# hwwang55/GraphGAN

Hardware: NVIDIA H100
Metric: sampled negative edges/sec (D-sampling pass) (higher is better)
Workload: dtype f32

## Files before the change

### graphgan_b200/csrc/walk.cu

```cuda
#include <string.h>

#include "walk_common.cuh"

namespace gg {
namespace {

struct Rng {
    int mode;
    uint32_t k0, k1, tag;
    const double *stream;
    long long n_stream;
    long long cursor;
    int exhausted;
    __device__ __forceinline__ double draw(uint32_t root, uint32_t walk, uint32_t step) {
        if (mode == GG_RNG_PHILOX) {
            uint32_t a, b;
            philox4x32_10(root, walk, step, tag, k0, k1, a, b);
            return u53(a, b);
        }
        if (cursor >= n_stream) { exhausted = 1; return 0.0; }
        return stream[cursor++];
    }
};

// ... 260 lines not shown
#define GG_S1_SINGLES 65536
#endif
constexpr int S1_SINGLES = GG_S1_SINGLES, S1_CHUNK = 16;

template <int CPL>
__global__ void __launch_bounds__(WARPS_PER_CTA * 32, WALK_MIN_CTAS) step1_cdf_kernel(const __grid_constant__ gg_walk_desc d) {
    extern __shared__ __align__(16) unsigned char walk_smem[];
    const int lane = threadIdx.x & 31, wid = threadIdx.x >> 5;
    float *s_sc = reinterpret_cast<float *>(walk_smem + (size_t)wid * WALK_SMEM_PER_WARP);
    int *s_ids = reinterpret_cast<int *>(s_sc + SC_CAP);
    Stage stg;
    stg.buf = s_sc;
    stg.bar = reinterpret_cast<unsigned long long *>(s_ids + ID_CAP);
    stg.phase = 0u;
    stg.on = !d.no_tma && d.edge_score != nullptr;
    if (stg.on) {
        if (lane == 0) {
            mbar_init(stg.bar, 1);
            asm volatile("fence.mbarrier_init.release.cluster;" ::: "memory");
        }
        __syncwarp();
    }
    const long long gw = (long long)blockIdx.x * WARPS_PER_CTA + wid;
    const long long nwarps = (long long)gridDim.x * WARPS_PER_CTA;
    int *g_ids = reinterpret_cast<int *>(d.scratch) + (size_t)gw * 2 * (size_t)d.max_cand;
    float *g_sc = reinterpret_cast<float *>(g_ids + d.max_cand);
    unsigned long long rows_gathered = 0;
    unsigned int cyc[7] = {0, 0, 0, 0, 0, 0, 0};
    long long item = gw, sub = 0, sub_end = 0;
    const long long n_single = d.s1_nq < S1_SINGLES ? d.s1_nq : S1_SINGLES;
    const long long n_items = n_single + (d.s1_nq - n_single + S1_CHUNK - 1) / S1_CHUNK;
    for (;;) {
        long long pos;
        if (d.s1_order) {
            if (sub >= sub_end) {
                unsigned int it = 0;
                if (lane == 0) it = atomicAdd(d.work_counter, 1u);
                it = __shfl_sync(FULL, it, 0);
                if ((long long)it >= n_items) break;
                if ((long long)it < n_single) { sub = it; sub_end = sub + 1; }
                else { sub = n_single + ((long long)it - n_single) * S1_CHUNK; sub_end = sub + S1_CHUNK < d.s1_nq ? sub + S1_CHUNK : d.s1_nq; }
            }
            pos = __ldg(d.s1_order + sub);
            ++sub;
        } else {
            if (item >= d.s1_nq) break;
            pos = item;
            item += nwarps;
        }
        if (!s1_is_shared(d, pos)) continue;
        const int slot = __ldg(d.s1_slot + pos);
        const int root = d.roots[slot];
        const uint32_t *tb = d.tree_bits + (size_t)slot * (size_t)d.tree_words;
        const long long e = d.indptr[root] + (pos - __ldg(d.rq_ptr + slot));
        const int c = __ldg(d.adj + e);
        const bool inc_father = !d.for_d && !((d.d1_bits[e >> 5] >> (e & 31)) & 1u);
        int n; float m; int *ids; float *sc;
        build_list<CPL, UNR_S1>(d, tb, c, root, inc_father, s_ids, s_sc, g_ids, g_sc, lane, n, m, ids, sc, rows_gathered, cyc, stg);
        if (lane == 0) d.s1_n[pos] = n;
        if (n == 0) continue;
        const long long o = __ldg(d.s1_ptr + pos);
        for (int i = lane; i < n; i += 32) d.s1_ids[o + i] = ids[i];
        if (n > 1) cdf_store_raw<UNR_S1>(sc, n, m, d.s1_q + o, lane);
        __syncwarp();
    }
    if (lane == 0 && rows_gathered) atomicAdd(d.counters + GG_CNT_ROWS_GATHERED, rows_gathered);
}

struct FlatView {
    int4 *list[2];
    int4 *tail;
    int *hub;
    int *item_n;
    int *pool_ids;
    unsigned *ctr;
    int stride;
    int steps;
    unsigned long long *keys;
    int *owner;
    int *rec_slot;
    int *uniq;
    double *pool_cdf;
    unsigned long long tbl_mask;
};
constexpr int FLAT_MAX_STEPS = 14;
constexpr int FLAT_CTR_WORDS = 1 + 4 * (FLAT_MAX_STEPS + 2);
#define GG_FCTR(fv, s, k) ((fv).ctr + 1 + 4 * (s) + (k))
__device__ __forceinline__ int4 *level_list(const FlatView &fv, int s) { return (s & 1) ? fv.list[1] : fv.list[0]; }

#ifndef GG_SHARE_LEVELS
#define GG_SHARE_LEVELS 0x4
#endif
constexpr unsigned SHARE_LEVELS = (unsigned)(GG_SHARE_LEVELS) & ~3u;
__host__ __device__ constexpr bool level_shared(int s) { return s < 32 && ((SHARE_LEVELS >> s) & 1u); }
inline bool any_level_shared(int steps) { return steps >= 2 && (SHARE_LEVELS & ((steps >= 31 ? ~0u : ((2u << steps) - 1u)))) != 0; }

template <int CPL>
__global__ void __launch_bounds__(WARPS_PER_CTA * 32, WALK_MIN_CTAS) walk_kernel(const __grid_constant__ gg_walk_desc d,
                                                                                 const FlatView fv, const int tail_mode) {
    extern __shared__ __align__(16) unsigned char walk_smem[];
    const int lane = threadIdx.x & 31, wid = threadIdx.x >> 5;
    float *s_sc = reinterpret_cast<float *>(walk_smem + (size_t)wid * WALK_SMEM_PER_WARP);
    int *s_ids = reinterpret_cast<int *>(s_sc + SC_CAP);
    Stage stg;
    stg.buf = s_sc;
    stg.bar = reinterpret_cast<unsigned long long *>(s_ids + ID_CAP);
    stg.phase = 0u;
    stg.on = !d.no_tma && d.edge_score != nullptr;
    if (stg.on) {
        if (lane == 0) {
            mbar_init(stg.bar, 1);
            asm volatile("fence.mbarrier_init.release.cluster;" ::: "memory");
        }
        __syncwarp();
    }
    const long long gw = (long long)blockIdx.x * WARPS_PER_CTA + wid;
    int *g_ids = reinterpret_cast<int *>(d.scratch) + (size_t)gw * 2 * (size_t)d.max_cand;
    float *g_sc = reinterpret_cast<float *>(g_ids + d.max_cand);
    Rng rng;
    rng.mode = GG_RNG_PHILOX; rng.k0 = (uint32_t)d.seed; rng.k1 = (uint32_t)(d.seed >> 32); rng.tag = d.pass_tag;
    rng.stream = nullptr; rng.n_stream = 0; rng.cursor = 0; rng.exhausted = 0;
    unsigned long long raw_steps = 0, raw_suml = 0, overflow = 0, rows_gathered = 0;
    unsigned int cyc[7] = {0, 0, 0, 0, 0, 0, 0};
    const bool ratio_all = d.update_ratio >= 1.0;

    const long long n_items = tail_mode ? (long long)fv.ctr[0] : d.n_walks;
    for (;;) {
        unsigned int wi = 0;
        if (lane == 0) wi = atomicAdd(d.work_counter, 1u);
        wi = __shfl_sync(FULL, wi, 0);
        if ((long long)wi >= n_items) break;
        if (tail_mode) {
            const int4 rec = fv.tail[wi];
            const long long w = rec.x;
            const int slot = rec.w;
            WalkState from;
            from.cur = rec.y; from.prev = rec.z; from.step = d.wsteps[w]; from.fedge = d.first_edge[w]; from.suml = d.wsuml[w];
            walk_one<CPL>(d, rng, slot, (uint32_t)(w - __ldg(d.walk_ptr + slot)), w, s_ids, s_sc, g_ids, g_sc, lane, raw_steps,
                          raw_suml, overflow, rows_gathered, cyc, stg, &from);
            continue;
        }
        const long long w = d.walk_order ? (long long)__ldg(d.walk_order + wi) : (long long)wi;
        int slot;
        if (d.walk_slot) {
            slot = __ldg(d.walk_slot + w);
        } else {
            long long lo = 0, hi = d.n_roots;
            while (hi - lo > 1) {
                const long long mid = (lo + hi) >> 1;
                if (__ldg(d.walk_ptr + mid) <= w) lo = mid; else hi = mid;
            }
            slot = (int)lo;
        }
        const uint32_t k = (uint32_t)(w - __ldg(d.walk_ptr + slot));
        if (!ratio_all) {
            uint32_t a, b;
            philox4x32_10((uint32_t)d.roots[slot], 0xffffffffu, 0u, rng.tag, rng.k0, rng.k1, a, b);
            if (!(u53(a, b) < d.update_ratio)) {
                if (lane == 0) {
                    d.samples[w] = -1; d.status[w] = GG_SKIPPED; d.first_edge[w] = -1; d.wsteps[w] = 0; d.wsuml[w] = 0;
                    if (d.path_len) d.path_len[w] = 0;
                }
                continue;
            }
        }
        walk_one<CPL>(d, rng, slot, k, w, s_ids, s_sc, g_ids, g_sc, lane, raw_steps, raw_suml, overflow, rows_gathered,
                      cyc, stg);
    }
    if (lane == 0) {
#pragma unroll
        for (int q = 0; q < 7; ++q) if (cyc[q]) atomicAdd(d.counters + GG_CNT_CYC_ENUM + q, (unsigned long long)cyc[q]);
        if (raw_steps) atomicAdd(d.counters + GG_CNT_RAW_STEPS, raw_steps);
        if (raw_suml) atomicAdd(d.counters + GG_CNT_RAW_SUML, raw_suml);
        if (overflow) atomicAdd(d.counters + GG_CNT_PATH_OVERFLOW, overflow);
        if (rows_gathered) atomicAdd(d.counters + GG_CNT_ROWS_GATHERED, rows_gathered);
    }
}

// ... 54 lines not shown
                status = GG_VOID;
            } else {
                const long long a0 = d.indptr[root];
                const int n0 = (int)(d.indptr[root + 1] - a0);
                fedge = (int)(a0 + fi);
                const int c = __ldg(d.adj + fedge);
                if (prow && 1 < d.max_path) prow[1] = c;
                ws = 1; wl = n0; steps = 1; suml = (unsigned)n0;
                const long long s1pos = __ldg(d.rq_ptr + slot) + fi;
                if (s1_is_shared(d, s1pos)) {
                    const int n = __ldg(d.s1_n + s1pos);
                    if (n == 0) {
                        status = GG_VOID;
                    } else {
                        const bool inc_father = step_includes_father(d, 1, fedge);
                        const long long o = __ldg(d.s1_ptr + s1pos);
                        uint32_t a, b;
                        philox4x32_10((uint32_t)root, k, 1u, d.pass_tag, (uint32_t)d.seed, (uint32_t)(d.seed >> 32), a, b);
                        const int idx = (n == 1) ? 0 : cdf_search_raw(d.s1_q + o, n, u53(a, b));
                        const int nxt = __ldg(d.s1_ids + o + idx);
                        if (prow && 2 < d.max_path) prow[2] = nxt;
                        ws = 2; wl = n0 + n; steps = 2; suml = (unsigned)(n0 + n);
                        if (inc_father && idx == 0) {
                            sample = c; status = GG_DONE; plen = 3;
                            if (d.max_path > 0 && 3 > d.max_path) over = 1;
                        } else {
                            rec = make_int4((int)w, nxt, c, slot); dest = 2;
                        }
                    }
                } else {
                    rec = make_int4((int)w, c, root, slot); dest = 1;
                }
            }
        }
        d.samples[w] = sample; d.status[w] = status; d.first_edge[w] = fedge; d.wsteps[w] = ws; d.wsuml[w] = wl;
        if (d.path_len) d.path_len[w] = plen;
    }
#pragma unroll
    for (int lv = 1; lv <= 2; ++lv) {
        const unsigned mk = __ballot_sync(FULL, dest == lv);
        if (!mk) continue;
        const int leader = __ffs(mk) - 1;
        int4 *list = (lv <= fv.steps) ? fv.list[lv & 1] : fv.tail;
        unsigned *cnt = (lv <= fv.steps) ? GG_FCTR(fv, lv, 0) : fv.ctr;
        unsigned base = 0;
        if (lane == leader) base = atomicAdd(cnt, (unsigned)__popc(mk));
        base = __shfl_sync(FULL, base, leader);
        if (dest == lv) list[base + __popc(mk & ((1u << lane) - 1u))] = rec;
    }
    steps = __reduce_add_sync(FULL, steps); suml = __reduce_add_sync(FULL, suml); over = __reduce_add_sync(FULL, over);
    if (lane == 0) {
        if (steps) atomicAdd(d.counters + GG_CNT_RAW_STEPS, (unsigned long long)steps);
        if (suml) atomicAdd(d.counters + GG_CNT_RAW_SUML, (unsigned long long)suml);
        if (over) atomicAdd(d.counters + GG_CNT_PATH_OVERFLOW, (unsigned long long)over);
    }
}

__device__ __forceinline__ unsigned long long share_hash(unsigned long long key, unsigned long long mask) {
    return ((key * 0x9E3779B97F4A7C15ull) >> 20) & mask;
}

template <class T>
__device__ __forceinline__ void warp_append(bool take, T *list, unsigned *cnt, const T &v, int lane) {
    const unsigned mk = __ballot_sync(FULL, take);
    if (!mk) return;
    const int leader = __ffs(mk) - 1;
    unsigned base = 0;
    if (lane == leader) base = atomicAdd(cnt, (unsigned)__popc(mk));
    base = __shfl_sync(FULL, base, leader);
    if (take) list[base + __popc(mk & ((1u << lane) - 1u))] = v;
}

__global__ void __launch_bounds__(256) flat_dedupe_kernel(const __grid_constant__ gg_walk_desc d, const FlatView fv, const int s) {
    const unsigned i = blockIdx.x * blockDim.x + threadIdx.x;
    const int lane = threadIdx.x & 31;
    const unsigned nA = *GG_FCTR(fv, s, 0);
    if (blockIdx.x * blockDim.x >= nA) return;
    bool hub = false, owner = false;
    if (i < nA) {
        const int4 rec = level_list(fv, s)[i];
        const int cur = rec.y, slot = rec.w;
        hub = d.edge_score && (d.indptr[cur + 1] - d.indptr[cur]) >= d.hub_threshold;
        int h = -1;
        if (!hub) {
            const unsigned long long key = (unsigned long long)slot * (unsigned long long)d.n_node + (unsigned long long)cur;
            unsigned long long p = share_hash(key, fv.tbl_mask);
            for (;;) {
                const unsigned long long old = atomicCAS(fv.keys + p, ~0ull, key);
                if (old == ~0ull) { owner = true; fv.owner[p] = (int)i; break; }
                if (old == key) break;
                p = (p + 1) & fv.tbl_mask;
            }
            h = (int)p;
        }
        fv.rec_slot[i] = h;
    }
    const int item = (int)i;
    warp_append(hub, fv.hub, GG_FCTR(fv, s, 1), item, lane);
    warp_append(owner, fv.uniq, GG_FCTR(fv, s, 2), item, lane);
}

__global__ void __launch_bounds__(256) flat_draw_kernel(const __grid_constant__ gg_walk_desc d, const FlatView fv, const int s) {
    const unsigned i = blockIdx.x * blockDim.x + threadIdx.x;
    const int lane = threadIdx.x & 31;
    const unsigned nA = *GG_FCTR(fv, s, 0);
    if (blockIdx.x * blockDim.x >= nA) return;
    unsigned long long overflow = 0;
    unsigned steps = 0, suml = 0;
    bool go_on = false;
    int4 rec = make_int4(0, 0, 0, 0);
    if (i < nA) {
        const int h = fv.rec_slot[i];
        if (h >= 0) {
            rec = level_list(fv, s)[i];
            const long long w = rec.x;
            const int cur = rec.y, slot = rec.w;
            const int item = fv.owner[h];
            const int nrec = fv.item_n[item];
            const int n = nrec & 0x3fffffff;
            if (n == 0) {
                flat_void(d, s, w);
            } else {
                const bool inc_father = (nrec >> 30) & 1;
                int idx = 0;
                if (n > 1) {
                    uint32_t a, b;
                    philox4x32_10((uint32_t)d.roots[slot], (uint32_t)(w - __ldg(d.walk_ptr + slot)), (uint32_t)s, d.pass_tag,
                                  (uint32_t)d.seed, (uint32_t)(d.seed >> 32), a, b);
                    idx = cdf_search_raw(fv.pool_cdf + (size_t)item * (size_t)(fv.stride + 1), n, u53(a, b));
                }
                const int nxt = fv.pool_ids[(size_t)item * (size_t)fv.stride + idx];
                go_on = flat_record_choice(d, s, w, cur, n, idx, nxt, inc_father, overflow);
                rec = make_int4((int)w, nxt, cur, slot);
                steps = 1; suml = (unsigned)n;
            }
        }
    }
    if (s < fv.steps) warp_append(go_on, level_list(fv, s + 1), GG_FCTR(fv, s + 1, 0), rec, lane);
    else warp_append(go_on, fv.tail, fv.ctr, rec, lane);
    steps = __reduce_add_sync(FULL, steps); suml = __reduce_add_sync(FULL, suml);
    const unsigned over = __reduce_add_sync(FULL, (unsigned)overflow);
    if (lane == 0) {
        if (steps) atomicAdd(d.counters + GG_CNT_RAW_STEPS, (unsigned long long)steps);
        if (suml) atomicAdd(d.counters + GG_CNT_RAW_SUML, (unsigned long long)suml);
        if (over) atomicAdd(d.counters + GG_CNT_PATH_OVERFLOW, (unsigned long long)over);
    }
}

constexpr int FLAT_ENUM_WARPS = 8;
template <bool SHARED>
__global__ void __launch_bounds__(FLAT_ENUM_WARPS * 32, 6) flat_enum_kernel(const __grid_constant__ gg_walk_desc d,
                                                                            const FlatView fv, const int s) {
    const int lane = threadIdx.x & 31;
    const unsigned gw = blockIdx.x * FLAT_ENUM_WARPS + (threadIdx.x >> 5), nwarps = gridDim.x * FLAT_ENUM_WARPS;
    const int4 *A = level_list(fv, s);
    const unsigned nA = SHARED ? *GG_FCTR(fv, s, 2) : *GG_FCTR(fv, s, 0);
    Stage stg;
    stg.buf = nullptr; stg.bar = nullptr; stg.phase = 0u; stg.on = false;
    unsigned long long raw_steps = 0, raw_suml = 0, overflow = 0;
    int4 rec_next = (gw < nA) ? A[SHARED ? fv.uniq[gw] : gw] : make_int4(0, 0, 0, 0);
    for (unsigned j = gw; j < nA; j += nwarps) {
        const unsigned i = SHARED ? (unsigned)fv.uniq[j] : j;
        const int4 rec = rec_next;
        if (j + nwarps < nA) rec_next = A[SHARED ? fv.uniq[j + nwarps] : j + nwarps];
        const long long w = rec.x;
        const int cur = rec.y, prev = rec.z, slot = rec.w;
        const long long a0 = d.indptr[cur], a1 = d.indptr[cur + 1];
        if (!SHARED && d.edge_score && (a1 - a0) >= d.hub_threshold) {
            if (lane == 0) { fv.hub[atomicAdd(GG_FCTR(fv, s, 1), 1u)] = (int)i; fv.item_n[i] = 0; }
            continue;
        }
        const bool inc_father = step_includes_father(d, s, s == 1 ? d.first_edge[w] : 0);
        const uint32_t *tb = d.tree_bits + (size_t)slot * (size_t)d.tree_words;
        int *ids = fv.pool_ids + (size_t)i * (size_t)fv.stride;
        int n = 0;
        if (inc_father) { if (lane == 0) ids[0] = prev; n = 1; }
        float m = 0.0f;
        enumerate_children<UNR>(d, tb, a0, a1, false, ids, nullptr, lane, n, m, stg);
        __syncwarp();
        if (SHARED) {
            if (lane == 0) fv.item_n[i] = n | (inc_father ? (1 << 30) : 0);
        } else if (n == 0) {
            if (lane == 0) { flat_void(d, s, w); fv.item_n[i] = 0; }
        } else if (n == 1) {
            const int nxt = inc_father ? prev : ids[0];
            if (lane == 0) { flat_advance(d, fv, s, w, slot, cur, 1, 0, nxt, inc_father, overflow); fv.item_n[i] = 0; }
            raw_steps += 1; raw_suml += 1;
        } else if (lane == 0) {
            fv.item_n[i] = n | (inc_father ? (1 << 30) : 0);
        }
    }
    if (lane == 0) {
        if (raw_steps) atomicAdd(d.counters + GG_CNT_RAW_STEPS, raw_steps);
        if (raw_suml) atomicAdd(d.counters + GG_CNT_RAW_SUML, raw_suml);
        if (overflow) atomicAdd(d.counters + GG_CNT_PATH_OVERFLOW, overflow);
    }
}

template <int CPL, bool SHARED>
__global__ void __launch_bounds__(WARPS_PER_CTA * 32, WALK_MIN_CTAS) flat_choose_kernel(const __grid_constant__ gg_walk_desc d,
                                                                                        const FlatView fv, const int s) {
    extern __shared__ __align__(16) unsigned char walk_smem[];
    const int lane = threadIdx.x & 31, wid = threadIdx.x >> 5;
    float *s_sc = reinterpret_cast<float *>(walk_smem + (size_t)wid * WALK_SMEM_PER_WARP);
    int *s_ids = reinterpret_cast<int *>(s_sc + SC_CAP);
    Stage stg;
    stg.buf = s_sc;
    stg.bar = reinterpret_cast<unsigned long long *>(s_ids + ID_CAP);
    stg.phase = 0u;
    stg.on = !d.no_tma && d.edge_score != nullptr;
    if (stg.on) {
        if (lane == 0) {
            mbar_init(stg.bar, 1);
            asm volatile("fence.mbarrier_init.release.cluster;" ::: "memory");
        }
        __syncwarp();
    }
    const long long gw = (long long)blockIdx.x * WARPS_PER_CTA + wid;
    int *g_ids = reinterpret_cast<int *>(d.scratch) + (size_t)gw * 2 * (size_t)d.max_cand;
    float *g_sc = reinterpret_cast<float *>(g_ids + d.max_cand);
    const int4 *A = level_list(fv, s);
    const unsigned nA = SHARED ? *GG_FCTR(fv, s, 2) : *GG_FCTR(fv, s, 0), nH = *GG_FCTR(fv, s, 1);
    const uint32_t k0 = (uint32_t)d.seed, k1 = (uint32_t)(d.seed >> 32);
    unsigned long long raw_steps = 0, raw_suml = 0, overflow = 0, rows_gathered = 0;
    unsigned int cyc[7] = {0, 0, 0, 0, 0, 0, 0};
    constexpr unsigned FLAT_CHUNK = 8;
    const unsigned n_pulls = nH + (nA + FLAT_CHUNK - 1) / FLAT_CHUNK;
    for (;;) {
        unsigned j = 0;
        if (lane == 0) j = atomicAdd(GG_FCTR(fv, s, 3), 1u);
        j = __shfl_sync(FULL, j, 0);
        if (j >= n_pulls) break;
        const bool hub_item = j < nH;
        unsigned p = hub_item ? 0u : (j - nH) * FLAT_CHUNK;
        const unsigned p_end = hub_item ? 1u : ((p + FLAT_CHUNK < nA) ? p + FLAT_CHUNK : nA);
        unsigned i_next = hub_item ? (unsigned)fv.hub[j] : (SHARED ? (unsigned)fv.uniq[p] : p);
        int4 rec_next = A[i_next];
        int n_next = hub_item ? 0 : fv.item_n[i_next];
        for (; p < p_end; ++p) {
            const unsigned i = i_next;
            const int4 rec = rec_next;
            const int nrec = n_next;
            if (p + 1 < p_end) {
                i_next = SHARED ? (unsigned)fv.uniq[p + 1] : p + 1;
                rec_next = A[i_next]; n_next = fv.item_n[i_next];
            }
            if (!hub_item && (nrec & 0x3fffffff) < 2) continue;
            const long long w = rec.x;
            const int cur = rec.y, prev = rec.z, slot = rec.w;
            int n, idx, nxt;
            bool inc_father;
            uint32_t a, b;
            if (hub_item) {
                inc_father = step_includes_father(d, s, s == 1 ? d.first_edge[w] : 0);
                const uint32_t *tb = d.tree_bits + (size_t)slot * (size_t)d.tree_words;
                int *ids; float *sc; float m;
                build_list<CPL, UNR>(d, tb, cur, prev, inc_father, s_ids, s_sc, g_ids, g_sc, lane, n, m, ids, sc, rows_gathered, cyc, stg);
                if (n == 0) {
                    if (lane == 0) flat_void(d, s, w);
                    continue;
                }
                philox4x32_10((uint32_t)d.roots[slot], (uint32_t)(w - __ldg(d.walk_ptr + slot)), (uint32_t)s, d.pass_tag, k0, k1, a, b);
                idx = (n == 1) ? 0 : choose_index(sc, n, m, u53(a, b), lane, sc != s_sc ? reinterpret_cast<double *>(s_sc) : nullptr);
                nxt = ids[idx];
                __syncwarp();
            } else {
                n = nrec & 0x3fffffff;
                inc_father = (nrec >> 30) & 1;
                const int *ids = fv.pool_ids + (size_t)i * (size_t)fv.stride;
                float4 c4[CPL];
                load_row<CPL>(d.emb, d.ld, cur, lane & 7, c4);
                const int root = d.roots[slot];
                const uint32_t k = (uint32_t)(w - __ldg(d.walk_ptr + slot));
                score_list<CPL>(d.emb, d.bias, d.ld, c4, ids, s_sc, n, cur, lane);
                rows_gathered += 1u + (unsigned)n;
                const float m = list_max(s_sc, n, lane);
                if (SHARED) {
                    cdf_store_raw<UNR>(s_sc, n, m, fv.pool_cdf + (size_t)i * (size_t)(fv.stride + 1), lane);
                    __syncwarp();
                    continue;
                }
                philox4x32_10((uint32_t)root, k, (uint32_t)s, d.pass_tag, k0, k1, a, b);
                idx = choose_index(s_sc, n, m, u53(a, b), lane);
                nxt = ids[idx];
                __syncwarp();
            }
            if (lane == 0) {
                flat_advance(d, fv, s, w, slot, cur, n, idx, nxt, inc_father, overflow);
                raw_steps += 1; raw_suml += (unsigned)n;
            }
        }
    }
    if (lane == 0) {
        if (raw_steps) atomicAdd(d.counters + GG_CNT_RAW_STEPS, raw_steps);
        if (raw_suml) atomicAdd(d.counters + GG_CNT_RAW_SUML, raw_suml);
        if (overflow) atomicAdd(d.counters + GG_CNT_PATH_OVERFLOW, overflow);
        if (rows_gathered) atomicAdd(d.counters + GG_CNT_ROWS_GATHERED, rows_gathered);
    }
}

size_t flat_layout(void *buf, long long n_walks, int hub_threshold, int steps, FlatView *fv) {
    const size_t W = (size_t)(n_walks > 0 ? n_walks : 1);
    const int stride = ((hub_threshold > 0 ? hub_threshold : 1) + 31) / 32 * 32;
    size_t off = 0;
    auto take = [&](size_t bytes) {
        void *p = buf ? (void *)((unsigned char *)buf + off) : nullptr;
        off += (bytes + 255) & ~(size_t)255;
        return p;
    };
    unsigned *ctr = (unsigned *)take(sizeof(unsigned) * FLAT_CTR_WORDS);
    int4 *l0 = (int4 *)take(16 * W), *l1 = (int4 *)take(16 * W), *tail = (int4 *)take(16 * W);
    int *hub = (int *)take(4 * W), *item_n = (int *)take(4 * W);
    int *pool = (int *)take(4 * W * (size_t)stride);
    unsigned long long cap = 0;
    unsigned long long *keys = nullptr;
    int *owner = nullptr, *rec_slot = nullptr, *uniq = nullptr;
    double *cdf = nullptr;
    if (any_level_shared(steps)) {
        cap = 1;
        while (cap < 2 * (unsigned long long)W) cap <<= 1;
        keys = (unsigned long long *)take(8 * cap);
        owner = (int *)take(4 * cap);
        rec_slot = (int *)take(4 * W);
        uniq = (int *)take(4 * W);
        cdf = (double *)take(8 * W * (size_t)(stride + 1));
    }
    if (fv) {
        fv->ctr = ctr; fv->list[0] = l0; fv->list[1] = l1; fv->tail = tail; fv->hub = hub;
        fv->item_n = item_n; fv->pool_ids = pool; fv->stride = stride; fv->steps = steps;
        fv->keys = keys; fv->owner = owner; fv->rec_slot = rec_slot; fv->uniq = uniq; fv->pool_cdf = cdf;
        fv->tbl_mask = cap ? cap - 1 : 0;
    }
    return off;
}

template <int CPL>
__global__ void __launch_bounds__(32) walk_stream_kernel(const __grid_constant__ gg_walk_desc d) {
    extern __shared__ __align__(16) unsigned char walk_smem[];
    float *s_sc = reinterpret_cast<float *>(walk_smem);
    int *s_ids = reinterpret_cast<int *>(s_sc + SC_CAP);
    const int lane = threadIdx.x;
    int *g_ids = reinterpret_cast<int *>(d.scratch);
    float *g_sc = reinterpret_cast<float *>(g_ids + d.max_cand);
    Rng rng;
    rng.mode = GG_RNG_STREAM; rng.k0 = rng.k1 = rng.tag = 0;
    rng.stream = d.stream; rng.n_stream = d.n_stream; rng.cursor = 0; rng.exhausted = 0;
    unsigned long long raw_steps = 0, raw_suml = 0, overflow = 0, rows_gathered = 0;
    unsigned int cyc[7] = {0, 0, 0, 0, 0, 0, 0};
    Stage stg;
    stg.buf = s_sc; stg.bar = nullptr; stg.phase = 0u; stg.on = false;
    for (long long slot = 0; slot < d.n_roots && !rng.exhausted; ++slot) {
        const long long w0 = d.walk_ptr[slot], w1 = d.walk_ptr[slot + 1];
        const double ur = rng.draw(0, 0, 0);
        const bool skip = !(ur < d.update_ratio);
        bool dead = skip || rng.exhausted;
        for (long long w = w0; w < w1; ++w) {
            if (dead) {
                if (lane == 0) {
                    d.samples[w] = -1; d.status[w] = skip ? GG_SKIPPED : GG_NOTRUN; d.first_edge[w] = -1;
                    d.wsteps[w] = 0; d.wsuml[w] = 0;
                    if (d.path_len) d.path_len[w] = 0;
                }
                continue;
            }
            const int st = walk_one<CPL>(d, rng, (int)slot, (uint32_t)(w - w0), w, s_ids, s_sc, g_ids, g_sc, lane,
                                         raw_steps, raw_suml, overflow, rows_gathered, cyc, stg);
            if (st != GG_DONE) dead = true;
        }
    }
    if (lane == 0) {
        atomicAdd(d.counters + GG_CNT_RAW_STEPS, raw_steps);
        atomicAdd(d.counters + GG_CNT_RAW_SUML, raw_suml);
        atomicAdd(d.counters + GG_CNT_PATH_OVERFLOW, overflow);
        atomicAdd(d.counters + GG_CNT_ROWS_GATHERED, rows_gathered);
        d.counters[GG_CNT_STREAM_USED] = (unsigned long long)rng.cursor + (rng.exhausted ? (1ull << 62) : 0ull);
    }
}

constexpr int FIN_NONE = 0x7f7f7f7f;

__device__ __forceinline__ long long walk_root_slot(const long long *__restrict__ walk_ptr, long long n_roots, long long w) {
    long long lo = 0, hi = n_roots;
    while (hi - lo > 1) {
        const long long mid = (lo + hi) >> 1;
        if (__ldg(walk_ptr + mid) <= w) lo = mid; else hi = mid;
    }
    return lo;
}

__global__ void finalize_mark_kernel(long long n_roots, const long long *__restrict__ walk_ptr, const int *__restrict__ status,
                                     int *root_ok) {
    const long long W = walk_ptr[n_roots];
    for (long long w = (long long)blockIdx.x * blockDim.x + threadIdx.x; w < W; w += (long long)gridDim.x * blockDim.x) {
        if (status[w] == GG_DONE) continue;
        const long long slot = walk_root_slot(walk_ptr, n_roots, w);
        atomicMin(root_ok + slot, (int)(w - walk_ptr[slot]));
    }
}

__global__ void finalize_apply_kernel(long long n_roots, const long long *__restrict__ walk_ptr, int for_d, int *samples,
                                      int *status, const int *__restrict__ first_edge, int *wsteps, int *wsuml, int *path_len,
                                      uint32_t *d1_bits, const int *__restrict__ root_ok, unsigned long long *counters) {
    const long long W = walk_ptr[n_roots];
    unsigned long long steps = 0, suml = 0;
    for (long long w = (long long)blockIdx.x * blockDim.x + threadIdx.x; w < W; w += (long long)gridDim.x * blockDim.x) {
        const long long slot = walk_root_slot(walk_ptr, n_roots, w);
        const long long off = w - walk_ptr[slot];
        if (off <= (long long)root_ok[slot]) {
            steps += (unsigned)wsteps[w]; suml += (unsigned)wsuml[w];
            if (for_d && status[w] == GG_DONE) {
                const int fe = first_edge[w];
                if (fe >= 0) atomicOr(d1_bits + (fe >> 5), 1u << (fe & 31));
            }
        } else {
// ... 71 lines not shown
    *bytes = (int64_t)gg::flat_layout(nullptr, n_walks, hub_threshold, flat_steps, nullptr);
    return 0;
}

extern "C" int gg_walk_sample(const gg_walk_desc *dp, void *stream) {
    GG_REQUIRE(dp, "null descriptor");
    const gg_walk_desc &d = *dp;
    GG_REQUIRE(d.ld > 0 && d.ld % 32 == 0, "ld must be a positive multiple of 32");
    if (d.n_walks == 0 || d.n_roots == 0) return 0;
    GG_REQUIRE(d.emb && d.bias && d.indptr && d.adj && d.roots && d.tree_bits && d.walk_ptr, "null graph/embedding pointer");
    GG_REQUIRE(d.tree_words > 0, "tree_words missing (gg_tree_words)");
    GG_REQUIRE(d.samples && d.status && d.first_edge && d.wsteps && d.wsuml && d.counters && d.work_counter,
               "null output pointer");
    GG_REQUIRE(d.for_d || d.d1_bits, "G mode needs d1_bits");
    GG_REQUIRE(d.n_walks < (1ll << 32), "too many walks in one call");
    GG_REQUIRE(d.max_cand > 0 && d.scratch, "scratch missing");
    GG_REQUIRE(!d.root_q || d.rq_ptr, "root_q needs rq_ptr");
    GG_REQUIRE(d.max_path >= 0 && (d.max_path == 0 || (d.paths && d.path_len)), "max_path > 0 needs paths and path_len");
    GG_REQUIRE(d.phase_mask >= 0 && d.phase_mask <= 3, "phase_mask must be 0..3");
    GG_REQUIRE(d.update_ratio >= 0.0, "update_ratio must be >= 0");
    GG_REQUIRE(d.rng_mode == GG_RNG_PHILOX || d.rng_mode == GG_RNG_STREAM, "unknown rng_mode");
    {
        const bool any_s1 = d.s1_q || d.s1_ids || d.s1_cnt || d.s1_n || d.s1_ptr || d.s1_slot || d.first_idx || d.s1_order;
        GG_REQUIRE(!any_s1 || (d.s1_q && d.s1_ids && d.s1_cnt && d.s1_n && d.s1_ptr && d.s1_slot && d.first_idx && d.s1_nq > 0),
                   "depth-1 reuse: s1_q, s1_ids, s1_cnt, s1_n, s1_ptr, s1_slot, first_idx and s1_nq go together");
        GG_REQUIRE(!any_s1 || d.rng_mode == GG_RNG_PHILOX, "depth-1 reuse needs GG_RNG_PHILOX");
        GG_REQUIRE(!d.walk_order || d.rng_mode == GG_RNG_PHILOX, "walk_order needs GG_RNG_PHILOX");
    }
    GG_REQUIRE(!d.edge_score || (d.hub_threshold > 0 && d.hub_threshold < gg::SMEM_CAP), "hub_threshold out of range");
    cudaStream_t st = (cudaStream_t)stream;
    GG_CHECK(cudaMemsetAsync(d.work_counter, 0, sizeof(unsigned int), st));
    if (d.n_walks == 0 || d.n_roots == 0) return 0;
    const int cpl = d.ld / 32;
    if (d.rng_mode == GG_RNG_STREAM) {
        GG_REQUIRE(d.stream, "stream mode needs the uniform stream");
        GG_REQUIRE(d.scratch_bytes >= 2ll * d.max_cand * 4, "scratch too small");
        switch (cpl) {
#define GG_STREAM(C)                                                                                                  \
    GG_CHECK(cudaFuncSetAttribute(gg::walk_stream_kernel<C>, cudaFuncAttributeMaxDynamicSharedMemorySize,            \
                                  gg::WALK_SMEM_PER_WARP));                                                          \
    gg::walk_stream_kernel<C><<<1, 32, gg::WALK_SMEM_PER_WARP, st>>>(d)
            case 1: GG_STREAM(1); break;
            case 2: GG_STREAM(2); break;
            case 4: GG_STREAM(4); break;
            case 8: GG_STREAM(8); break;
#undef GG_STREAM
            default: gg::set_error("gg_walk_sample: unsupported ld %d (supported: 32, 64, 128, 256)", d.ld); return 2;
        }
    } else {
        const int ctas = gg::grid_ctas();
        GG_REQUIRE(d.scratch_bytes >= (int64_t)ctas * gg::WARPS_PER_CTA * 2 * d.max_cand * 4, "scratch too small");
        const int pm = d.phase_mask ? d.phase_mask : 3;
        if (d.s1_q && (pm & 1)) {
            GG_REQUIRE(d.root_q && d.walk_slot && d.first_idx && d.s1_cnt && d.s1_n && d.s1_ptr && d.s1_ids && d.s1_slot,
                       "depth-1 reuse needs root_q, walk_slot and the s1_* buffers");
            GG_CHECK(cudaMemsetAsync(d.s1_cnt, 0, sizeof(int32_t) * (size_t)d.s1_nq, st));
            gg::root_step_kernel<<<(unsigned)((d.n_walks + 255) / 256), 256, 0, st>>>(d);
            GG_CHECK(cudaGetLastError());
#define GG_S1(C)                                                                                                      \
    GG_CHECK(cudaFuncSetAttribute(gg::step1_cdf_kernel<C>, cudaFuncAttributeMaxDynamicSharedMemorySize,              \
                                  gg::WARPS_PER_CTA * gg::WALK_SMEM_PER_WARP));                                      \
    gg::step1_cdf_kernel<C><<<ctas, gg::WARPS_PER_CTA * 32, gg::WARPS_PER_CTA * gg::WALK_SMEM_PER_WARP, st>>>(d)
            switch (cpl) {
                case 1: GG_S1(1); break;
                case 2: GG_S1(2); break;
                case 4: GG_S1(4); break;
                case 8: GG_S1(8); break;
                default: gg::set_error("gg_walk_sample: unsupported ld %d (supported: 32, 64, 128, 256)", d.ld); return 2;
            }
#undef GG_S1
            GG_CHECK(cudaGetLastError());
            GG_CHECK(cudaMemsetAsync(d.work_counter, 0, sizeof(unsigned int), st));
        }
        if (!(pm & 2)) return 0;
        gg::FlatView fv;
        memset(&fv, 0, sizeof(fv));
        int tail_mode = 0;
        if (d.flat_steps > 0) {
            GG_REQUIRE(d.s1_q && d.edge_score && d.root_q && d.walk_slot && d.first_idx, "flat_steps needs the depth-1 reuse (s1_*, edge_score, root_q, walk_slot)");
            GG_REQUIRE(d.flat_steps <= gg::FLAT_MAX_STEPS, "flat_steps too large");
            GG_REQUIRE(d.flat_buf && d.flat_bytes >= (int64_t)gg::flat_layout(nullptr, d.n_walks, d.hub_threshold, d.flat_steps, nullptr),
                       "flat_buf too small (gg_walk_flat_bytes)");
            gg::flat_layout(d.flat_buf, d.n_walks, d.hub_threshold, d.flat_steps, &fv);
            GG_CHECK(cudaMemsetAsync(fv.ctr, 0, sizeof(unsigned) * gg::FLAT_CTR_WORDS, st));
            gg::flat_start_kernel<<<(unsigned)((d.n_walks + 255) / 256), 256, 0, st>>>(d, fv);
            GG_CHECK(cudaGetLastError());
            const int enum_ctas = gg::sm_count() * 8;
            const unsigned rec_ctas = (unsigned)((d.n_walks + 255) / 256);
            GG_REQUIRE(!gg::any_level_shared(d.flat_steps) || d.n_node > 0, "n_node missing");
            for (int s = 1; s <= d.flat_steps; ++s) {
                const bool shared = gg::level_shared(s);
                if (shared) {
                    GG_CHECK(cudaMemsetAsync(fv.keys, 0xff, sizeof(unsigned long long) * (size_t)(fv.tbl_mask + 1), st));
                    gg::flat_dedupe_kernel<<<rec_ctas, 256, 0, st>>>(d, fv, s);
                    GG_CHECK(cudaGetLastError());
                    gg::flat_enum_kernel<true><<<enum_ctas, gg::FLAT_ENUM_WARPS * 32, 0, st>>>(d, fv, s);
                } else {
                    gg::flat_enum_kernel<false><<<enum_ctas, gg::FLAT_ENUM_WARPS * 32, 0, st>>>(d, fv, s);
                }
                GG_CHECK(cudaGetLastError());
                switch (cpl) {
#define GG_FLAT(C)                                                                                                    \
    if (shared) {                                                                                                    \
        GG_CHECK(cudaFuncSetAttribute(gg::flat_choose_kernel<C, true>, cudaFuncAttributeMaxDynamicSharedMemorySize,  \
                                      gg::WARPS_PER_CTA * gg::WALK_SMEM_PER_WARP));                                  \
        gg::flat_choose_kernel<C, true><<<ctas, gg::WARPS_PER_CTA * 32, gg::WARPS_PER_CTA * gg::WALK_SMEM_PER_WARP, st>>>(d, fv, s); \
    } else {                                                                                                         \
        GG_CHECK(cudaFuncSetAttribute(gg::flat_choose_kernel<C, false>, cudaFuncAttributeMaxDynamicSharedMemorySize, \
                                      gg::WARPS_PER_CTA * gg::WALK_SMEM_PER_WARP));                                  \
        gg::flat_choose_kernel<C, false><<<ctas, gg::WARPS_PER_CTA * 32, gg::WARPS_PER_CTA * gg::WALK_SMEM_PER_WARP, st>>>(d, fv, s); \
    }
                    case 1: GG_FLAT(1); break;
                    case 2: GG_FLAT(2); break;
                    case 4: GG_FLAT(4); break;
                    case 8: GG_FLAT(8); break;
#undef GG_FLAT
                    default: gg::set_error("gg_walk_sample: unsupported ld %d (supported: 32, 64, 128, 256)", d.ld); return 2;
                }
                GG_CHECK(cudaGetLastError());
                if (shared) {
                    gg::flat_draw_kernel<<<rec_ctas, 256, 0, st>>>(d, fv, s);
                    GG_CHECK(cudaGetLastError());
                }
            }
            tail_mode = 1;
        }
        switch (cpl) {
#define GG_WALK(C)                                                                                                    \
    GG_CHECK(cudaFuncSetAttribute(gg::walk_kernel<C>, cudaFuncAttributeMaxDynamicSharedMemorySize,                   \
                                  gg::WARPS_PER_CTA * gg::WALK_SMEM_PER_WARP));                                      \
    gg::walk_kernel<C><<<ctas, gg::WARPS_PER_CTA * 32, gg::WARPS_PER_CTA * gg::WALK_SMEM_PER_WARP, st>>>(d, fv, tail_mode)
            case 1: GG_WALK(1); break;
            case 2: GG_WALK(2); break;
            case 4: GG_WALK(4); break;
            case 8: GG_WALK(8); break;
#undef GG_WALK
            default: gg::set_error("gg_walk_sample: unsupported ld %d (supported: 32, 64, 128, 256)", d.ld); return 2;
        }
    }
    return gg::check_cuda(cudaGetLastError(), "walk kernel launch");
}

extern "C" int gg_walk_finalize(int64_t n_roots, const int64_t *walk_ptr, int32_t for_d, int32_t *samples,
                                int32_t *status, const int32_t *first_edge, int32_t *wsteps, int32_t *wsuml,
                                int32_t *path_len, uint32_t *d1_bits, int32_t *root_ok,
                                unsigned long long *counters, void *stream) {
    GG_REQUIRE(walk_ptr && samples && status && first_edge && wsteps && wsuml && root_ok && counters, "null pointer");
    GG_REQUIRE(!for_d || d1_bits, "D mode needs d1_bits");
    if (n_roots == 0) return 0;
    cudaStream_t st = (cudaStream_t)stream;
    const int threads = 256;
    const unsigned wgrid = (unsigned)(gg::sm_count() * 8);
    GG_CHECK(cudaMemsetAsync(root_ok, 0x7f, sizeof(int32_t) * (size_t)n_roots, st));
    gg::finalize_mark_kernel<<<wgrid, threads, 0, st>>>(n_roots, (const long long *)walk_ptr, status, root_ok);
    GG_CHECK(cudaGetLastError());
    gg::finalize_apply_kernel<<<wgrid, threads, 0, st>>>(n_roots, (const long long *)walk_ptr, for_d, samples, status, first_edge,
                                                        wsteps, wsuml, path_len, d1_bits, root_ok, counters);
    GG_CHECK(cudaGetLastError());
    gg::finalize_roots_kernel<<<(unsigned)((n_roots + threads - 1) / threads), threads, 0, st>>>(
        n_roots, (const long long *)walk_ptr, root_ok, counters);
    return gg::check_cuda(cudaGetLastError(), "finalize kernel launch");
}

extern "C" int gg_emit_d_rows(int64_t n_roots, const int32_t *roots, const int64_t *walk_ptr,
                              const int64_t *pos_indptr, const int32_t *pos_flat, const int32_t *root_ok,
                              const int32_t *samples, int64_t *row_ptr, int32_t *center, int32_t *neighbor,
                              int32_t *label, int64_t *n_rows_out, void *stream) {
    GG_REQUIRE(row_ptr && n_rows_out, "null pointer");
    GG_REQUIRE(n_roots == 0 || (roots && walk_ptr && pos_indptr && pos_flat && root_ok && samples), "null pointer");
    cudaStream_t st = (cudaStream_t)stream;
    const int threads = 256;
    if (n_roots > 0) {
        gg::row_count_kernel<<<(unsigned)((n_roots + threads - 1) / threads), threads, 0, st>>>(
            n_roots, (const long long *)walk_ptr, root_ok, (long long *)row_ptr);
        GG_CHECK(cudaGetLastError());
    }
    int rc = gg::launch_exclusive_scan_i64((long long *)row_ptr, n_roots, (long long *)n_rows_out, st);
    if (rc) return rc;
// ... 9 lines not shown
```

### graphgan_b200/csrc/walk_common.cuh

```cuda
#pragma once
#include "gg_common.cuh"

namespace gg {

#ifndef GG_SC_CAP
#define GG_SC_CAP 2048
#endif
#ifndef GG_UNR
#define GG_UNR 4
#endif
#ifndef GG_UNR_S1
#define GG_UNR_S1 8
#endif
#ifndef GG_WALK_MIN_CTAS
#define GG_WALK_MIN_CTAS 3
#endif
constexpr int WARPS_PER_CTA = 8;
constexpr int WALK_MIN_CTAS = GG_WALK_MIN_CTAS;
constexpr int ID_CAP = 320;
constexpr int SC_CAP = GG_SC_CAP;
constexpr int SMEM_CAP = ID_CAP;
constexpr int WALK_SMEM_PER_WARP = SC_CAP * 4 + ID_CAP * 4 + 16;
constexpr int STAGE_ENTRIES = 512;
static_assert(2 * STAGE_ENTRIES * 4 <= SC_CAP * 4, "the staging area is the warp's (idle) score buffer");
// ... 124 lines not shown
            double x = (double)__fdiv_rn(e[u], S);
            x = warp_scan_ks(x, lane);
            total = __dadd_rn(total, __shfl_sync(FULL, x, 31));
            const int t = (t0 >> 5) + u;
            if (t < 64 && lane == (t & 31)) car[t >> 5] = total;
        }
    }
    return total;
}

__device__ __forceinline__ int cdf_pick_from(const float *sc, int n, float S, double total, double u, int lane,
                                             int t_begin, double carry) {
    for (int t0 = 32 * t_begin; t0 < n; t0 += 32) {
        const int i = t0 + lane;
        double x = (double)__fdiv_rn((i < n) ? sc[i] : 0.0f, S);
        x = warp_scan_ks(x, lane);
        const double q = __ddiv_rn(__dadd_rn(carry, x), total);
        const unsigned hit = __ballot_sync(FULL, (i < n) && (q > u));
        if (hit) return t0 + __ffs(hit) - 1;
        carry = __dadd_rn(carry, __shfl_sync(FULL, x, 31));
    }
    return n - 1;
}

__device__ __forceinline__ int cdf_pick(const float *sc, int n, float S, double total, double u, int lane,
                                        const double (&car)[2]) {
    const int ntiles = (n + 31) >> 5;
    int t_hit = -1;
#pragma unroll
    for (int h = 0; h < 2; ++h) {
        const int t = 32 * h + lane;
        const bool p = (t < ntiles) && (__ddiv_rn(car[h], total) > u);
        const unsigned mk = __ballot_sync(FULL, p);
        if (t_hit < 0 && mk) t_hit = 32 * h + __ffs(mk) - 1;
    }
    if (t_hit < 0) {
        if (ntiles <= 64) return n - 1;
        const double c63 = __shfl_sync(FULL, car[1], 31);
        return cdf_pick_from(sc, n, S, total, u, lane, 64, c63);
    }
    double before = 0.0;
    if (t_hit > 0) {
        const int tp = t_hit - 1;
        const double lo = __shfl_sync(FULL, car[0], tp & 31), hi = __shfl_sync(FULL, car[1], tp & 31);
        before = (tp >> 5) ? hi : lo;
    }
    return cdf_pick_from(sc, n, S, total, u, lane, t_hit, before);
}

__device__ __forceinline__ double cdf_total_tiles(const float *sc, int n, float S, int lane, double *tiles) {
    constexpr int U = 8;
    double total = 0.0;
    for (int t0 = 0; t0 < n; t0 += 32 * U) {
        float e[U];
#pragma unroll
        for (int u = 0; u < U; ++u) { const int i = t0 + 32 * u + lane; e[u] = (i < n) ? sc[i] : 0.0f; }
#pragma unroll
        for (int u = 0; u < U; ++u) {
            if (t0 + 32 * u >= n) break;
            double x = (double)__fdiv_rn(e[u], S);
            x = warp_scan_ks(x, lane);
            total = __dadd_rn(total, __shfl_sync(FULL, x, 31));
            if (lane == 0) tiles[(t0 >> 5) + u] = total;
        }
    }
    __syncwarp();
    return total;
}
__device__ __forceinline__ int cdf_pick_tiles(const float *sc, int n, float S, double total, double u, int lane,
                                              const double *tiles) {
    const int ntiles = (n + 31) >> 5;
    for (int tb = 0; tb < ntiles; tb += 32) {
        const int t = tb + lane;
        const bool p = (t < ntiles) && (__ddiv_rn(tiles[t], total) > u);
        const unsigned mk = __ballot_sync(FULL, p);
        if (mk) {
            const int t_hit = tb + __ffs(mk) - 1;
            return cdf_pick_from(sc, n, S, total, u, lane, t_hit, t_hit > 0 ? tiles[t_hit - 1] : 0.0);
        }
    }
    return n - 1;
}

static __device__ __noinline__ int choose_index_long(float *sc, int n, float m, double u, int lane, double *tiles) {
    float S;
    double car[2], total;
    if (tiles && ((n + 31) >> 5) <= SC_CAP / 2) {
        S = softmax_exp_sum<8>(sc, n, m, lane);
        total = cdf_total_tiles(sc, n, S, lane, tiles);
        return cdf_pick_tiles(sc, n, S, total, u, lane, tiles);
    }
    S = softmax_exp_sum<8>(sc, n, m, lane);
    total = cdf_total<8>(sc, n, S, lane, car);
    return cdf_pick(sc, n, S, total, u, lane, car);
}

__device__ __forceinline__ int choose_index(float *sc, int n, float m, double u, int lane, double *tiles = nullptr) {
    if (n <= 32) {
        const float e = (lane < n) ? exp_c(__fsub_rn(sc[lane], m)) : 0.0f;
        const float S = warp_sum_butterfly(e);
        const double x = warp_scan_ks((double)__fdiv_rn(e, S), lane);
        const double total = __shfl_sync(FULL, x, 31);
        const unsigned hit = __ballot_sync(FULL, (lane < n) && (__ddiv_rn(x, total) > u));
        return hit ? __ffs(hit) - 1 : n - 1;
    }
    if (n > SC_CAP) return choose_index_long(sc, n, m, u, lane, tiles);
    double car[2];
    const float S = softmax_exp_sum(sc, n, m, lane);
    const double total = cdf_total(sc, n, S, lane, car);
    return cdf_pick(sc, n, S, total, u, lane, car);
}

__device__ __forceinline__ void cdf_store(float *sc, int n, double *q_out, int lane) {
    const float m = list_max(sc, n, lane);
    const float S = softmax_exp_sum<UNR_S1>(sc, n, m, lane);
    double car[2];
    const double total = cdf_total<UNR_S1>(sc, n, S, lane, car);
    double carry = 0.0;
    for (int t0 = 0; t0 < n; t0 += 32) {
        const int i = t0 + lane;
        double x = (i < n) ? (double)__fdiv_rn(sc[i], S) : 0.0;
        x = warp_scan_ks(x, lane);
        if (i < n) q_out[i] = __ddiv_rn(__dadd_rn(carry, x), total);
        carry = __dadd_rn(carry, __shfl_sync(FULL, x, 31));
    }
}

template <int U>
__device__ __forceinline__ void cdf_store_raw(float *sc, int n, float m, double *c_out, int lane) {
    const float S = softmax_exp_sum<U>(sc, n, m, lane);
    double carry = 0.0;
    for (int t0 = 0; t0 < n; t0 += 32 * U) {
        double x[U];
#pragma unroll
        for (int u = 0; u < U; ++u) {
            const int i = t0 + 32 * u + lane;
            x[u] = (i < n) ? (double)__fdiv_rn(sc[i], S) : 0.0;
        }
#pragma unroll
        for (int u = 0; u < U; ++u) x[u] = warp_scan_ks(x[u], lane);
#pragma unroll
        for (int u = 0; u < U; ++u) {
            if (t0 + 32 * u >= n) break;
            const int i = t0 + 32 * u + lane;
            if (i < n) c_out[i] = __dadd_rn(carry, x[u]);
            carry = __dadd_rn(carry, __shfl_sync(FULL, x[u], 31));
        }
    }
    if (lane == 0) c_out[n] = carry;
}

__device__ __forceinline__ int cdf_search_raw(const double *__restrict__ c, int n, double u) {
    const double total = __ldg(c + n);
    int lo = 0, hi = n - 1;
    while (lo < hi) {
        const int mid = (lo + hi) >> 1;
        if (__ddiv_rn(__ldg(c + mid), total) > u) hi = mid; else lo = mid + 1;
    }
    return lo;
}

__device__ __forceinline__ int cdf_search(const double *__restrict__ q, int n, double u) {
    int lo = 0, hi = n - 1;
    while (lo < hi) {
        const int mid = (lo + hi) >> 1;
        if (__ldg(q + mid) > u) hi = mid; else lo = mid + 1;
    }
    return lo;
}

}
```

Measured before the change: 98.79 million.

## Share hub-node candidate lists across walks with identical (slot, node) keys

Hub records are now deduplicated by (slot, current node) in the existing hash table. Each hub group gets one build_list and CDF preparation, and every walk in the group draws from that shared CDF. Two new kernels count group sizes, reserve work items of up to 128 walks, and scatter record indices into the groups. This removes repeated construction and softmax of large hub neighbour lists, at the cost of extra launches, atomics, a serial per-walk draw loop inside each warp, and possible load imbalance.

```diff
diff --git a/graphgan_b200/csrc/walk.cu b/graphgan_b200/csrc/walk.cu
--- a/graphgan_b200/csrc/walk.cu
+++ b/graphgan_b200/csrc/walk.cu
@@ -366,10 +366,16 @@
     int *uniq;
     double *pool_cdf;
     unsigned long long tbl_mask;
+    unsigned *gcnt;
+    unsigned *gpos;
+    int *hub_rec;
+    int4 *hub_work;
 };
 constexpr int FLAT_MAX_STEPS = 14;
 constexpr int FLAT_CTR_WORDS = 1 + 4 * (FLAT_MAX_STEPS + 2);
+constexpr int FLAT_CTR_ALL = FLAT_CTR_WORDS + 3 * (FLAT_MAX_STEPS + 2);
 #define GG_FCTR(fv, s, k) ((fv).ctr + 1 + 4 * (s) + (k))
+#define GG_FCTR_HUB(fv, s, k) ((fv).ctr + FLAT_CTR_WORDS + 3 * (s) + (k))
 __device__ __forceinline__ int4 *level_list(const FlatView &fv, int s) { return (s & 1) ? fv.list[1] : fv.list[0]; }
 
 #ifndef GG_SHARE_LEVELS
@@ -378,6 +384,16 @@
 constexpr unsigned SHARE_LEVELS = (unsigned)(GG_SHARE_LEVELS) & ~3u;
 __host__ __device__ constexpr bool level_shared(int s) { return s < 32 && ((SHARE_LEVELS >> s) & 1u); }
 inline bool any_level_shared(int steps) { return steps >= 2 && (SHARE_LEVELS & ((steps >= 31 ? ~0u : ((2u << steps) - 1u)))) != 0; }
+
+#ifndef GG_SHARE_HUB
+#define GG_SHARE_HUB 1
+#endif
+#ifndef GG_HUB_GROUP_MAX
+#define GG_HUB_GROUP_MAX 128
+#endif
+constexpr bool SHARE_HUB = GG_SHARE_HUB != 0;
+constexpr int HUB_GROUP_MAX = GG_HUB_GROUP_MAX;
+static_assert(HUB_GROUP_MAX > 0 && HUB_GROUP_MAX % 32 == 0, "hub work items are whole warps of walks");
 
 template <int CPL>
 __global__ void __launch_bounds__(WARPS_PER_CTA * 32, WALK_MIN_CTAS) walk_kernel(const __grid_constant__ gg_walk_desc d,
@@ -598,7 +614,7 @@
         const int cur = rec.y, slot = rec.w;
         hub = d.edge_score && (d.indptr[cur + 1] - d.indptr[cur]) >= d.hub_threshold;
         int h = -1;
-        if (!hub) {
+        if (!hub || SHARE_HUB) {
             const unsigned long long key = (unsigned long long)slot * (unsigned long long)d.n_node + (unsigned long long)cur;
             unsigned long long p = share_hash(key, fv.tbl_mask);
             for (;;) {
@@ -608,12 +624,65 @@
                 p = (p + 1) & fv.tbl_mask;
             }
             h = (int)p;
+            if (hub) {
+                atomicAdd(fv.gcnt + p, 1u);
+                h = -2 - h;
+            }
         }
         fv.rec_slot[i] = h;
     }
     const int item = (int)i;
-    warp_append(hub, fv.hub, GG_FCTR(fv, s, 1), item, lane);
-    warp_append(owner, fv.uniq, GG_FCTR(fv, s, 2), item, lane);
+    if (SHARE_HUB) {
+        const unsigned mk = __ballot_sync(FULL, hub);
+        if (lane == 0 && mk) atomicAdd(GG_FCTR(fv, s, 1), (unsigned)__popc(mk));
+        warp_append(hub && owner, fv.hub, GG_FCTR_HUB(fv, s, 0), item, lane);
+    } else {
+        warp_append(hub, fv.hub, GG_FCTR(fv, s, 1), item, lane);
+    }
+    warp_append(owner && !hub, fv.uniq, GG_FCTR(fv, s, 2), item, lane);
+}
+
+__device__ __forceinline__ unsigned warp_reserve(unsigned v, unsigned *cnt, int lane) {
+    unsigned incl = v;
+#pragma unroll
+    for (int off = 1; off < 32; off <<= 1) {
+        const unsigned x = __shfl_up_sync(FULL, incl, off);
+        if (lane >= off) incl += x;
+    }
+    unsigned base = 0;
+    if (lane == 31 && incl) base = atomicAdd(cnt, incl);
+    return __shfl_sync(FULL, base, 31) + incl - v;
+}
+
+__global__ void __launch_bounds__(256) flat_hub_reserve_kernel(const FlatView fv, const int s) {
+    const unsigned j = blockIdx.x * blockDim.x + threadIdx.x;
+    const int lane = threadIdx.x & 31;
+    const unsigned nO = *GG_FCTR_HUB(fv, s, 0);
+    if (blockIdx.x * blockDim.x >= nO) return;
+    int orec = 0;
+    unsigned p = 0, cnt = 0, nw = 0;
+    if (j < nO) {
+        orec = fv.hub[j];
+        p = (unsigned)(-2 - fv.rec_slot[orec]);
+        cnt = fv.gcnt[p];
+        nw = (cnt + HUB_GROUP_MAX - 1) / HUB_GROUP_MAX;
+    }
+    const unsigned base = warp_reserve(cnt, GG_FCTR_HUB(fv, s, 2), lane);
+    const unsigned it = warp_reserve(nw, GG_FCTR_HUB(fv, s, 1), lane);
+    if (j < nO) {
+        fv.gpos[p] = base;
+        for (unsigned q = 0; q < nw; ++q) {
+            const unsigned first = q * HUB_GROUP_MAX;
+            fv.hub_work[it + q] = make_int4(orec, (int)(base + first), (int)min(cnt - first, (unsigned)HUB_GROUP_MAX), 0);
+        }
+    }
+}
+
+__global__ void __launch_bounds__(256) flat_hub_fill_kernel(const FlatView fv, const int s) {
+    const unsigned i = blockIdx.x * blockDim.x + threadIdx.x;
+    if (i >= *GG_FCTR(fv, s, 0)) return;
+    const int h = fv.rec_slot[i];
+    if (h <= -2) fv.hub_rec[atomicAdd(fv.gpos + (-2 - h), 1u)] = (int)i;
 }
 
 __global__ void __launch_bounds__(256) flat_draw_kernel(const __grid_constant__ gg_walk_desc d, const FlatView fv, const int s) {
@@ -736,7 +805,9 @@
     int *g_ids = reinterpret_cast<int *>(d.scratch) + (size_t)gw * 2 * (size_t)d.max_cand;
     float *g_sc = reinterpret_cast<float *>(g_ids + d.max_cand);
     const int4 *A = level_list(fv, s);
-    const unsigned nA = SHARED ? *GG_FCTR(fv, s, 2) : *GG_FCTR(fv, s, 0), nH = *GG_FCTR(fv, s, 1);
+    constexpr bool GROUPS = SHARED && SHARE_HUB;
+    const unsigned nA = SHARED ? *GG_FCTR(fv, s, 2) : *GG_FCTR(fv, s, 0);
+    const unsigned nH = GROUPS ? *GG_FCTR_HUB(fv, s, 1) : *GG_FCTR(fv, s, 1);
     const uint32_t k0 = (uint32_t)d.seed, k1 = (uint32_t)(d.seed >> 32);
     unsigned long long raw_steps = 0, raw_suml = 0, overflow = 0, rows_gathered = 0;
     unsigned int cyc[7] = {0, 0, 0, 0, 0, 0, 0};
@@ -748,6 +819,51 @@
         j = __shfl_sync(FULL, j, 0);
         if (j >= n_pulls) break;
         const bool hub_item = j < nH;
+        if (GROUPS && hub_item) {
+            const int4 hw = fv.hub_work[j];
+            const int4 orec = A[hw.x];
+            const int cur = orec.y, prev = orec.z, slot = orec.w;
+            const int root = d.roots[slot];
+            const long long wp = __ldg(d.walk_ptr + slot);
+            int w_lane = (lane < hw.z) ? A[fv.hub_rec[hw.y + lane]].x : 0;
+            const uint32_t *tb = d.tree_bits + (size_t)slot * (size_t)d.tree_words;
+            int n; float m; int *ids; float *sc;
+            build_list<CPL, UNR>(d, tb, cur, prev, true, s_ids, s_sc, g_ids, g_sc, lane, n, m, ids, sc, rows_gathered, cyc, stg);
+            double *tiles = sc != s_sc ? reinterpret_cast<double *>(s_sc) : nullptr;
+            ListCdf cdf;
+            if (n >= 2) cdf_prepare(sc, n, m, lane, tiles, cdf);
+            unsigned long long ov = 0;
+            for (int q0 = 0; q0 < hw.z; q0 += 32) {
+                if (q0) w_lane = (q0 + lane < hw.z) ? A[fv.hub_rec[hw.y + q0 + lane]].x : 0;
+                const int nq = min(32, hw.z - q0);
+                const bool mine = lane < nq;
+                int idx = 0;
+                if (n >= 2) {
+                    uint32_t a, b;
+                    philox4x32_10((uint32_t)root, (uint32_t)(w_lane - wp), (uint32_t)s, d.pass_tag, k0, k1, a, b);
+                    const double u_lane = u53(a, b);
+                    for (int t = 0; t < nq; ++t) {
+                        const int it = cdf_draw(sc, n, cdf, __shfl_sync(FULL, u_lane, t), lane, tiles);
+                        if (lane == t) idx = it;
+                    }
+                }
+                bool go_on = false;
+                int4 next = make_int4(0, 0, 0, 0);
+                if (mine && n == 0) flat_void(d, s, w_lane);
+                if (mine && n > 0) {
+                    const int nxt = ids[idx];
+                    go_on = flat_record_choice(d, s, w_lane, cur, n, idx, nxt, true, ov);
+                    next = make_int4(w_lane, nxt, cur, slot);
+                }
+                if (s < fv.steps) warp_append(go_on, level_list(fv, s + 1), GG_FCTR(fv, s + 1, 0), next, lane);
+                else warp_append(go_on, fv.tail, fv.ctr, next, lane);
+                if (lane == 0 && n > 0) { raw_steps += (unsigned)nq; raw_suml += (unsigned)nq * (unsigned)n; }
+            }
+            const unsigned ovw = __reduce_add_sync(FULL, (unsigned)ov);
+            if (lane == 0) overflow += ovw;
+            __syncwarp();
+            continue;
+        }
         unsigned p = hub_item ? 0u : (j - nH) * FLAT_CHUNK;
         const unsigned p_end = hub_item ? 1u : ((p + FLAT_CHUNK < nA) ? p + FLAT_CHUNK : nA);
         unsigned i_next = hub_item ? (unsigned)fv.hub[j] : (SHARED ? (unsigned)fv.uniq[p] : p);
@@ -824,13 +940,15 @@
         off += (bytes + 255) & ~(size_t)255;
         return p;
     };
-    unsigned *ctr = (unsigned *)take(sizeof(unsigned) * FLAT_CTR_WORDS);
+    unsigned *ctr = (unsigned *)take(sizeof(unsigned) * FLAT_CTR_ALL);
     int4 *l0 = (int4 *)take(16 * W), *l1 = (int4 *)take(16 * W), *tail = (int4 *)take(16 * W);
     int *hub = (int *)take(4 * W), *item_n = (int *)take(4 * W);
     int *pool = (int *)take(4 * W * (size_t)stride);
     unsigned long long cap = 0;
     unsigned long long *keys = nullptr;
-    int *owner = nullptr, *rec_slot = nullptr, *uniq = nullptr;
+    int *owner = nullptr, *rec_slot = nullptr, *uniq = nullptr, *hub_rec = nullptr;
+    unsigned *gcnt = nullptr, *gpos = nullptr;
+    int4 *hub_work = nullptr;
     double *cdf = nullptr;
     if (any_level_shared(steps)) {
         cap = 1;
@@ -840,12 +958,19 @@
         rec_slot = (int *)take(4 * W);
         uniq = (int *)take(4 * W);
         cdf = (double *)take(8 * W * (size_t)(stride + 1));
+        if (SHARE_HUB) {
+            gcnt = (unsigned *)take(4 * cap);
+            gpos = (unsigned *)take(4 * cap);
+            hub_rec = (int *)take(4 * W);
+            hub_work = (int4 *)take(16 * W);
+        }
     }
     if (fv) {
         fv->ctr = ctr; fv->list[0] = l0; fv->list[1] = l1; fv->tail = tail; fv->hub = hub;
         fv->item_n = item_n; fv->pool_ids = pool; fv->stride = stride; fv->steps = steps;
         fv->keys = keys; fv->owner = owner; fv->rec_slot = rec_slot; fv->uniq = uniq; fv->pool_cdf = cdf;
         fv->tbl_mask = cap ? cap - 1 : 0;
+        fv->gcnt = gcnt; fv->gpos = gpos; fv->hub_rec = hub_rec; fv->hub_work = hub_work;
     }
     return off;
 }
@@ -1083,7 +1208,7 @@
             GG_REQUIRE(d.flat_buf && d.flat_bytes >= (int64_t)gg::flat_layout(nullptr, d.n_walks, d.hub_threshold, d.flat_steps, nullptr),
                        "flat_buf too small (gg_walk_flat_bytes)");
             gg::flat_layout(d.flat_buf, d.n_walks, d.hub_threshold, d.flat_steps, &fv);
-            GG_CHECK(cudaMemsetAsync(fv.ctr, 0, sizeof(unsigned) * gg::FLAT_CTR_WORDS, st));
+            GG_CHECK(cudaMemsetAsync(fv.ctr, 0, sizeof(unsigned) * gg::FLAT_CTR_ALL, st));
             gg::flat_start_kernel<<<(unsigned)((d.n_walks + 255) / 256), 256, 0, st>>>(d, fv);
             GG_CHECK(cudaGetLastError());
             const int enum_ctas = gg::sm_count() * 8;
@@ -1093,8 +1218,15 @@
                 const bool shared = gg::level_shared(s);
                 if (shared) {
                     GG_CHECK(cudaMemsetAsync(fv.keys, 0xff, sizeof(unsigned long long) * (size_t)(fv.tbl_mask + 1), st));
+                    if (gg::SHARE_HUB) GG_CHECK(cudaMemsetAsync(fv.gcnt, 0, sizeof(unsigned) * (size_t)(fv.tbl_mask + 1), st));
                     gg::flat_dedupe_kernel<<<rec_ctas, 256, 0, st>>>(d, fv, s);
                     GG_CHECK(cudaGetLastError());
+                    if (gg::SHARE_HUB) {
+                        gg::flat_hub_reserve_kernel<<<rec_ctas, 256, 0, st>>>(fv, s);
+                        GG_CHECK(cudaGetLastError());
+                        gg::flat_hub_fill_kernel<<<rec_ctas, 256, 0, st>>>(fv, s);
+                        GG_CHECK(cudaGetLastError());
+                    }
                     gg::flat_enum_kernel<true><<<enum_ctas, gg::FLAT_ENUM_WARPS * 32, 0, st>>>(d, fv, s);
                 } else {
                     gg::flat_enum_kernel<false><<<enum_ctas, gg::FLAT_ENUM_WARPS * 32, 0, st>>>(d, fv, s);
diff --git a/graphgan_b200/csrc/walk_common.cuh b/graphgan_b200/csrc/walk_common.cuh
--- a/graphgan_b200/csrc/walk_common.cuh
+++ b/graphgan_b200/csrc/walk_common.cuh
@@ -230,6 +230,35 @@
     return n - 1;
 }
 
+__device__ __forceinline__ double tile1_cdf(const float *sc, int n, float m, int lane, double &total) {
+    const float e = (lane < n) ? exp_c(__fsub_rn(sc[lane], m)) : 0.0f;
+    const float S = warp_sum_butterfly(e);
+    const double x = warp_scan_ks((double)__fdiv_rn(e, S), lane);
+    total = __shfl_sync(FULL, x, 31);
+    return x;
+}
+__device__ __forceinline__ int tile1_pick(double x, double total, int n, double u, int lane) {
+    const unsigned hit = __ballot_sync(FULL, (lane < n) && (__ddiv_rn(x, total) > u));
+    return hit ? __ffs(hit) - 1 : n - 1;
+}
+
+struct ListCdf {
+    float S;
+    double total;
+    double car[2];
+};
+
+__device__ __forceinline__ bool long_uses_tiles(int n, const double *tiles) { return tiles && ((n + 31) >> 5) <= SC_CAP / 2; }
+static __device__ __noinline__ void cdf_prepare_long(float *sc, int n, float m, int lane, double *tiles, ListCdf &c) {
+    c.S = softmax_exp_sum<8>(sc, n, m, lane);
+    if (long_uses_tiles(n, tiles)) c.total = cdf_total_tiles(sc, n, c.S, lane, tiles);
+    else c.total = cdf_total<8>(sc, n, c.S, lane, c.car);
+}
+static __device__ __noinline__ int cdf_draw_long(const float *sc, int n, const ListCdf &c, double u, int lane,
+                                                 const double *tiles) {
+    if (long_uses_tiles(n, tiles)) return cdf_pick_tiles(sc, n, c.S, c.total, u, lane, tiles);
+    return cdf_pick(sc, n, c.S, c.total, u, lane, c.car);
+}
 static __device__ __noinline__ int choose_index_long(float *sc, int n, float m, double u, int lane, double *tiles) {
     float S;
     double car[2], total;
@@ -243,14 +272,28 @@
     return cdf_pick(sc, n, S, total, u, lane, car);
 }
 
+__device__ __forceinline__ void cdf_prepare(float *sc, int n, float m, int lane, double *tiles, ListCdf &c) {
+    if (n <= 32) {
+        c.car[0] = tile1_cdf(sc, n, m, lane, c.total);
+    } else if (n > SC_CAP) {
+        cdf_prepare_long(sc, n, m, lane, tiles, c);
+    } else {
+        c.S = softmax_exp_sum(sc, n, m, lane);
+        c.total = cdf_total(sc, n, c.S, lane, c.car);
+    }
+}
+
+__device__ __forceinline__ int cdf_draw(const float *sc, int n, const ListCdf &c, double u, int lane, const double *tiles) {
+    if (n <= 32) return tile1_pick(c.car[0], c.total, n, u, lane);
+    if (n > SC_CAP) return cdf_draw_long(sc, n, c, u, lane, tiles);
+    return cdf_pick(sc, n, c.S, c.total, u, lane, c.car);
+}
+
 __device__ __forceinline__ int choose_index(float *sc, int n, float m, double u, int lane, double *tiles = nullptr) {
     if (n <= 32) {
-        const float e = (lane < n) ? exp_c(__fsub_rn(sc[lane], m)) : 0.0f;
-        const float S = warp_sum_butterfly(e);
-        const double x = warp_scan_ks((double)__fdiv_rn(e, S), lane);
-        const double total = __shfl_sync(FULL, x, 31);
-        const unsigned hit = __ballot_sync(FULL, (lane < n) && (__ddiv_rn(x, total) > u));
-        return hit ? __ffs(hit) - 1 : n - 1;
+        double total;
+        const double x = tile1_cdf(sc, n, m, lane, total);
+        return tile1_pick(x, total, n, u, lane);
     }
     if (n > SC_CAP) return choose_index_long(sc, n, m, u, lane, tiles);
     double car[2];
```

New measurement: 105.7 million (median of 6 runs). 7.0% higher.
